# minfenli/refnerf-pl

Measured on AMD Instinct MI355X. Metric: ray-samples/s (4096 rays x 128 samples x 2 levels, Ref-NeRF Blender, eval forward), higher is better.
Workload: dtype f16x2; 1 GPU; blender_refnerf.gin, 4096 rays x 128 samples, 2-level, Model.__call__ eval forward with compute_extras + full ray_history; rays_per_gpu=4096, total_rays=4096, samples_per_level=128, parallelism=ray-tile dp1, n_ranks_seen=1, hip_graph_replay=False

## Files before the change

refnerf-pl_amd/csrc/refnerf_level_bf16.h:

```cpp
#pragma once
#include <type_traits>

#include "refnerf_level_common.h"

namespace rn {

typedef short v2s __attribute__((ext_vector_type(2)));

struct MmBf16 {
  typedef __bf16 t;
  typedef t v8 __attribute__((ext_vector_type(8)));
  typedef t v2 __attribute__((ext_vector_type(2)));
  static __device__ __forceinline__ v16f mfma(v8 a, v8 b, v16f c) { return __builtin_amdgcn_mfma_f32_32x32x16_bf16(a, b, c, 0, 0, 0); }
};
struct MmF16 {
  typedef _Float16 t;
  typedef t v8 __attribute__((ext_vector_type(8)));
  typedef t v2 __attribute__((ext_vector_type(2)));
  static __device__ __forceinline__ v16f mfma(v8 a, v8 b, v16f c) { return __builtin_amdgcn_mfma_f32_32x32x16_f16(a, b, c, 0, 0, 0); }
};
template <typename MM>
__device__ __forceinline__ unsigned cvt_pk_mm(float lo, float hi) {
  typename MM::v2 r = __builtin_convertvector((v2f){lo, hi}, typename MM::v2);
  return __builtin_bit_cast(unsigned, r);
}
constexpr bool ENC_FAST = true;

constexpr int BT = 256;
constexpr int BF_NW = 8;
constexpr int BF_NTHREADS = 64 * BF_NW;
constexpr int BF_RING_SLOTS = 3;
constexpr int BF_RING_BYTES = BF_RING_SLOTS * BF_CHUNK_BYTES;
constexpr int BF_X_BYTES = (IPE_DIM / 8) * BT * 16;
constexpr int AF = 2;
static_assert(AF == 1 || AF == 2 || AF == 4, "the ring index k % AF must stay in phase across 8- and 16-step chunks, and the ring may only run into "
                                             "the next chunk after that chunk's rendezvous (8-step chunks: k >= 4)");

typedef __attribute__((address_space(1))) const void *gptr_t;
typedef __attribute__((address_space(3))) void *lptr_t;

struct Pipe {
  const char *sp;
  unsigned pos;
  unsigned lane_off;
  const char *src;
  const char *src_end;
  char *wbuf;
  const char *xp;
  const char *xps;
  int seq;
  int cur_off, nxt_off, fil_off;
  int dma_left;
  int lane, wave, h;
  long long t_vm, t_bar;
};

#ifdef REFNERF_PROF_WAITS
#define RN_RENDEZVOUS(p) do { \
    long long t0_ = (long long)__builtin_readcyclecounter(); \
    asm volatile("s_waitcnt vmcnt(0)" ::: "memory"); \
    long long t1_ = (long long)__builtin_readcyclecounter(); \
    __syncthreads(); \
    (p).t_vm += t1_ - t0_; \
    (p).t_bar += (long long)__builtin_readcyclecounter() - t1_; } while (0)
#else
#define RN_RENDEZVOUS(p) do { asm volatile("s_waitcnt vmcnt(0)" ::: "memory"); __syncthreads(); } while (0)
#endif
__device__ __forceinline__ void ring_rotate(Pipe &p) {
  const int t = p.cur_off;
  p.cur_off = p.nxt_off;
  p.nxt_off = p.fil_off;
  p.fil_off = t;
}
static_assert(SPPACKED.sp_chunks == 8 + 7 * 16 + 8 + 5 && SPPACKED.total_chunks - SPPACKED.sp_chunks == 8 + 7 * 8 + 8 + 1,
              "the places where level_fwd_split moves the stream position back are written for this chunk sequence");
constexpr int SP_ADV_REWIND = (1 - SPPACKED.sp_chunks) * BF_CHUNK_BYTES;
constexpr int SP_ADV_WRAP = (1 - SPPACKED.total_chunks) * BF_CHUNK_BYTES;
template <bool SPLIT = false>
__device__ __forceinline__ void issue_chunk(Pipe &p, int slot_off, int piece = -1, int adv = BF_CHUNK_BYTES) {
  if (p.dma_left <= 0) return;
  lptr_t dst = (lptr_t)(p.wbuf + slot_off + p.wave * 3072);
  asm volatile("" : "+v"(p.lane_off));
  gptr_t src = (gptr_t)((SPLIT ? p.sp : p.sp + p.pos) + p.lane_off);
  if (piece < 0 || piece == 0) __builtin_amdgcn_global_load_lds(src, dst, 16, 0, 0);
  if (piece < 0 || piece == 1) __builtin_amdgcn_global_load_lds(src, dst, 16, 1024, 0);
  if ((piece < 0 || piece == 2) && p.wave < 5) __builtin_amdgcn_global_load_lds(src, dst, 16, 2048, 0);
  if (piece >= 0 && piece < 2) return;
  p.dma_left -= 1;
  if constexpr (SPLIT) p.sp += adv;
  else {
    p.pos += BF_CHUNK_BYTES;
    p.pos = (p.pos == (unsigned)BFPACKED.chunks_per_pass * BF_CHUNK_BYTES) ? 0u : p.pos;
  }
}
__device__ __forceinline__ void pipe_stream_init(Pipe &p, const void *image, int chunks, int wave, int lane) {
  p.sp = reinterpret_cast<const char *>(image);
  p.pos = 0;
  p.lane_off = (unsigned)(wave * 3072 + lane * 16);
  p.dma_left = wave < 6 ? chunks : 0;
  p.src = nullptr; p.src_end = nullptr; p.seq = 0;
}

template <typename MM>
__device__ __forceinline__ typename MM::v8 lds_frag(const char *q) {
  return *reinterpret_cast<const typename MM::v8 *>(q);
}

__device__ __forceinline__ v16f bias16(const char *w, int h) {
  const v4f *bp = reinterpret_cast<const v4f *>(w + h * 64);
  v4f b0 = bp[0], b1 = bp[1], b2 = bp[2], b3 = bp[3];
  return (v16f){b0[0], b0[1], b0[2], b0[3], b1[0], b1[1], b1[2], b1[3],
                b2[0], b2[1], b2[2], b2[3], b3[0], b3[1], b3[2], b3[3]};
}

template <typename MM, bool RELU>
__device__ __forceinline__ unsigned pack_pair(float lo, float hi) {
  unsigned w = cvt_pk_mm<MM>(lo, hi);
  if (RELU) {
    v2s s = __builtin_bit_cast(v2s, w);
    s = __builtin_elementwise_max(s, (v2s){0, 0});
    w = __builtin_bit_cast(unsigned, s);
  }
  return w;
}

template <typename MM, bool RELU>
__device__ __forceinline__ void pack_acc(const v16f &a, v4uu &f0, v4uu &f1) {
#pragma unroll
  for (int e = 0; e < 4; ++e) {
    f0[e] = pack_pair<MM, RELU>(a[2 * e], a[2 * e + 1]);
    f1[e] = pack_pair<MM, RELU>(a[8 + 2 * e], a[8 + 2 * e + 1]);
  }
}

template <typename MM, int REAL>
__device__ __forceinline__ typename MM::v8 lds_b(const Pipe &p, int kl) {
  const int kk = (kl < REAL) ? kl : kl - REAL;
  return lds_frag<MM>(p.xp + (2 * kk) * BT * 16);
}

struct NoHook { __device__ __forceinline__ void operator()(int) const {} };
template <typename MM, int KIND, int REAL_L, bool FIRST, bool SPLIT = false, typename Hook = NoHook>
__device__ __forceinline__ void bf_chunk(Pipe &p, typename MM::v8 (&a)[AF], const v4uu (&in)[16], const v4uu (&bn)[8], v16f &acc, Hook &&hook = Hook(), int adv = BF_CHUNK_BYTES) {
  typedef typename MM::v8 v8mm;
  constexpr int KS = (KIND == BF_LDS8) ? 8 : 16;
  constexpr int L0 = (KIND == BF_BNLDS) ? 8 : 0;
  constexpr int RDV = KS / 2 - 1;
  static_assert(KS % AF == 0, "ring phase");
  const char *w = p.wbuf + p.cur_off;
  const char *cur = w + 1024 + p.lane * 16;
  const char *nxt = p.wbuf + p.nxt_off + 1024 + p.lane * 16;
  v8mm xr[2];
  if (KIND == BF_LDS8) { xr[0] = lds_b<MM, REAL_L>(p, 0); xr[1] = lds_b<MM, REAL_L>(p, 1); }
  if (FIRST) acc = bias16(w, p.h);
  __builtin_amdgcn_sched_barrier(0);
#pragma unroll
  for (int k = 0; k < KS; ++k) {
    v8mm b;
    const bool lds_step = (KIND == BF_LDS8) || (KIND == BF_BNLDS && k >= 8);
    if (lds_step) b = xr[(k - L0) & 1];
    else if (KIND == BF_REG) b = __builtin_bit_cast(v8mm, in[k]);
    else b = __builtin_bit_cast(v8mm, bn[k & 7]);
    acc = MM::mfma(a[k % AF], b, acc);
    a[k % AF] = (k + AF < KS) ? lds_frag<MM>(cur + (k + AF) * 1024) : lds_frag<MM>(nxt + (k + AF - KS) * 1024);
    hook(k);
    if (KIND == BF_LDS8 || KIND == BF_BNLDS) {
      const int kl2 = k + 2 - L0;
      if (kl2 >= 0 && kl2 < 8 && !(KIND == BF_LDS8 && kl2 < 2)) xr[kl2 & 1] = lds_b<MM, REAL_L>(p, kl2);
    }
    if (k == RDV) {
      RN_RENDEZVOUS(p);
      issue_chunk<SPLIT>(p, p.fil_off, 0);
    }
    if (k == RDV + 2) issue_chunk<SPLIT>(p, p.fil_off, 1);
    if (k == RDV + 4) issue_chunk<SPLIT>(p, p.fil_off, 2, adv);
    __builtin_amdgcn_sched_barrier(0);
  }
  ring_rotate(p);
}

template <bool SPLIT = false>
__device__ __forceinline__ void idle_pass(Pipe &p) {
#pragma unroll 1
  for (int c = 0; c < (SPLIT ? SPPACKED.chunks_per_pass : BFPACKED.chunks_per_pass); ++c) {
    RN_RENDEZVOUS(p);
    issue_chunk<SPLIT>(p, p.fil_off, -1, c + 3 == SPPACKED.sp_chunks ? SP_ADV_REWIND : (c + 3 == SPPACKED.chunks_per_pass ? SP_ADV_WRAP : BF_CHUNK_BYTES));
    ring_rotate(p);
  }
}

template <typename MM, int KIND0, int REAL0>
__device__ __forceinline__ void bf_slice(Pipe &p, typename MM::v8 (&a)[AF], int second, const v4uu (&in)[16], const v4uu (&bn)[8], v16f &acc) {
  bf_chunk<MM, KIND0, REAL0, true>(p, a, in, bn, acc);
  if constexpr (KIND0 == BF_REG) {
    if (second == 1) bf_chunk<MM, BF_LDS8, BF_IPE_REAL_KS, false>(p, a, in, bn, acc);
    else if (second == 2) bf_chunk<MM, BF_BNLDS, BF_DIR_REAL_KS, false>(p, a, in, bn, acc);
  }
}

template <typename MM, int KIND0, int REAL0>
__device__ __forceinline__ void bf_layer(Pipe &p, typename MM::v8 (&a)[AF], int second, const v4uu (&in)[16], const v4uu (&bn)[8], v4uu (&out)[16]) {
#pragma unroll
  for (int ob = 0; ob < 8; ++ob) {
    v16f acc;
    bf_slice<MM, KIND0, REAL0>(p, a, second, in, bn, acc);
    pack_acc<MM, true>(acc, out[2 * ob], out[2 * ob + 1]);
    __builtin_amdgcn_sched_barrier(0);
  }
}

#define RN_STAMPW(A, slot) do { asm volatile("; RNMARK " #slot); if ((A).prof && blockIdx.x == (gridDim.x >> 1) && lane == 0) (A).prof[wave * 32 + (slot)] = (long long)__builtin_readcyclecounter(); } while (0)

constexpr int BF_PS_RING = 512;
template <typename MM, bool RINGPS = false>
__device__ __forceinline__ void level_fwd_mm(const LevelArgs &A) {
  constexpr int PSM = RINGPS ? BF_PS_RING - 1 : 0;
  typedef typename MM::v8 v8mm;
  typedef typename MM::t mm_t;
  extern __shared__ __attribute__((aligned(16))) float smem[];
  const refnerf_level_cfg &cfg = A.cfg;
  const int N = cfg.n_samples;
  const int tid = threadIdx.x, lane = tid & 63;
  const int wave = __builtin_amdgcn_readfirstlane(tid >> 6);
  const int rpw = A.rpw;
  const int ray0 = blockIdx.x * rpw;
  const int n_tot = rpw * N;
  const int n_pass = (n_tot + BT - 1) / BT;

  char *WB = reinterpret_cast<char *>(smem);
  char *Xb = WB + BF_RING_BYTES;
  float *HD = reinterpret_cast<float *>(Xb + BF_X_BYTES);
  float *TD = HD + HD_ROWS * BT;
  float *XP = TD + rpw * (N + 1);
  float *PS = XP + rpw * (N + 1);
  float *PX = PS + (RINGPS ? BF_PS_RING : n_tot) * NPS_EVAL;
  float *NRM = PX + 3 * BT;
  const float *RY = NRM + 8;

  const int h = lane >> 5, n = lane & 31;
  const int col = wave * 32 + n;

  Pipe p;
  pipe_stream_init(p, A.packed, n_pass * BFPACKED.chunks_per_pass, wave, lane);
  p.wbuf = WB;
  p.xp = Xb + (h * BT + col) * 16;
  p.cur_off = 0; p.nxt_off = BF_CHUNK_BYTES; p.fil_off = 2 * BF_CHUNK_BYTES;
  p.lane = lane; p.wave = wave; p.h = h;
  p.t_vm = 0; p.t_bar = 0;
  RN_STAMPW(A, 0);
  issue_chunk(p, p.cur_off);
  issue_chunk(p, p.nxt_off);

  resample_phase<BF_NW, false>(A, reinterpret_cast<float *>(Xb), TD, NRM, ray0, wave, lane);
  RN_STAMPW(A, 1);
  asm volatile("s_waitcnt vmcnt(0)" ::: "memory");
  __syncthreads();
  RN_STAMPW(A, 2);

  if (wave >= BF_NW / 2) __builtin_amdgcn_s_setprio(1);
  v4uu R0[16], R1[16], bn[8];
  v8mm ar[AF];
#pragma unroll
  for (int d = 0; d < AF; ++d) ar[d] = lds_frag<MM>(WB + 1024 + lane * 16 + d * 1024);

  for (int pass0 = 0; pass0 < n_tot; pass0 += BT) {
    int lane_v = lane, col_v = col;
    asm volatile("" : "+v"(lane_v), "+v"(col_v));
    p.lane_off = (unsigned)(wave * 3072 + lane_v * 16);
    auto locate = [&](int &g, int &rl, int &si, bool &valid) {
      int col_l = col, pass_l = pass0;
      asm volatile("" : "+v"(col_l), "+s"(pass_l));
      g = pass_l + col_l;
      rl = g / N;
      si = g - rl * N;
      valid = (g < n_tot) && (ray0 + rl < A.R);
    };
    auto pass_epilogue = [&]() {
      if constexpr (RINGPS) {
        __syncthreads();
        const int end = (pass0 + BT < n_tot) ? pass0 + BT : n_tot;
        int td_o = (int)(TD - smem), xp_o = (int)(XP - smem), ps_o = (int)(PS - smem), nrm_o = (int)(NRM - smem), lane_e = lane, pass_e = pass0;
        int ntot_e = n_tot, ray0_e = ray0, wave_e = wave;
        asm volatile("" : "+s"(td_o), "+s"(xp_o), "+s"(ps_o), "+s"(nrm_o), "+v"(lane_e), "+s"(pass_e), "+s"(ntot_e), "+s"(ray0_e), "+s"(wave_e));
        composite_phase<BF_NW, true, NPS_EVAL, PSM>(A, smem + td_o, smem + xp_o, smem + ps_o, ntot_e, ray0_e, wave_e, lane_e, nullptr, smem + nrm_o,
                                                    pass_e / N, end / N);
      }
    };
    {
      const int g0 = pass0 + wave * 32;
      if (g0 >= n_tot || ray0 + g0 / N >= A.R) { idle_pass(p); pass_epilogue(); continue; }
    }
    auto load_heads = [&](SampleHeads &sh) {
      int g, rl, si; bool valid;
      locate(g, rl, si, valid);
      int ci = col, ro = (valid ? rl : 0) * 12;
      asm volatile("" : "+v"(ci), "+v"(ro));
      float v[3], gp[3], raw_dif[3], raw_tint[3];
#pragma unroll
      for (int i = 0; i < 3; ++i) {
        v[i] = RY[ro + 6 + i];
        gp[i] = HD[(1 + i) * BT + ci];
        raw_dif[i] = HD[(5 + i) * BT + ci];
        raw_tint[i] = HD[(8 + i) * BT + ci];
      }
      sample_heads<ENC_FAST>(cfg, HD[0 * BT + ci], gp, HD[4 * BT + ci], raw_dif, raw_tint, v, sh);
    };

#pragma unroll 1
    for (int phase = 0; phase < 2; ++phase) {
#pragma unroll
      for (int e = 0; e < 16; ++e) { R0[e] = (v4uu){0, 0, 0, 0}; R1[e] = (v4uu){0, 0, 0, 0}; }
      if (phase == 0) {
#pragma unroll
        for (int e = 0; e < 8; ++e) bn[e] = (v4uu){0, 0, 0, 0};
      }
      char *xs = Xb + col * 16;
      if (phase == 0) {
        int g, rl, si; bool valid;
        locate(g, rl, si, valid);
        float o[3], d[3];
        const float *ry = RY + (valid ? rl : 0) * 12;
#pragma unroll
        for (int i = 0; i < 3; ++i) { o[i] = ry[i]; d[i] = ry[3 + i]; }
        float radius = ry[9];
        const float *td = TD + (valid ? rl : 0) * (N + 1);
        float t0 = td[valid ? si : 0], t1 = td[valid ? si + 1 : 1];
        float lm[3], lv[3];
        cast_sample(o, d, radius, t0, t1, cfg.ray_shape, lm, lv);
        if (cfg.disable_integration) { lv[0] = 0.0f; lv[1] = 0.0f; lv[2] = 0.0f; }
        RN_STAMPW(A, 17);
#pragma unroll 1
        for (int qq = 0; qq < 2; ++qq) {
#pragma unroll
          for (int q = 0; q < 3; ++q) {
            v8mm pk;
#pragma unroll
            for (int e = 0; e < 8; ++e) {
              const int kk = q * 8 + e;
              pk[e] = (mm_t)ipe_feature<ENC_FAST>(lm[kk % 3], lv[kk % 3], 8 * qq + kk / 3, h);
            }
            *reinterpret_cast<v8mm *>(xs + (6 * h + 3 * qq + q) * BT * 16) = pk;
          }
        }
        RN_STAMPW(A, 18);
      } else {
        SampleHeads sh;
        load_heads(sh);
        float ide[40];
#pragma unroll
        for (int q = 36; q < 40; ++q) ide[q] = 0.0f;
        if (cfg.dir_enc == REFNERF_DIRENC_POSENC) posenc_eval<ENC_FAST>(sh.refd[0], sh.refd[1], sh.refd[2], h, [&](int q, float val) { ide[q] = val; });
        else ide_eval<ENC_FAST>(sh.refd[0], sh.refd[1], sh.refd[2], sh.rough, h, [&](int q, float val) { ide[q] = val; });
        if (h == 0) ide[36] = sh.dot;
#pragma unroll
        for (int q = 0; q < 5; ++q) {
          v8mm pk;
#pragma unroll
          for (int e = 0; e < 8; ++e) pk[e] = (mm_t)ide[q * 8 + e];
          *reinterpret_cast<v8mm *>(xs + (5 * h + q) * BT * 16) = pk;
        }
      }
      wave_sync();
      RN_STAMPW(A, 3 + phase * 8);

      if (phase == 0) bf_layer<MM, BF_LDS8, BF_IPE_REAL_KS>(p, ar, 0, R0, bn, R0);
      else bf_layer<MM, BF_BNLDS, BF_DIR_REAL_KS>(p, ar, 0, R0, bn, R0);
      RN_STAMPW(A, 4 + phase * 8);
#pragma unroll 1
      for (int it = 0; it < 4; ++it) {
        const int second = (it == 2) ? (phase ? 2 : 1) : 0;
        bf_layer<MM, BF_REG, 0>(p, ar, second, R0, bn, R1);
        if (it < 3) bf_layer<MM, BF_REG, 0>(p, ar, 0, R1, bn, R0);
      }
      RN_STAMPW(A, 5 + phase * 8);
      if (phase == 0) {
#pragma unroll
        for (int ob = 0; ob < 5; ++ob) {
          v16f acc;
          bf_slice<MM, BF_REG, 0>(p, ar, 0, R1, bn, acc);
          if (ob < 4) pack_acc<MM, false>(acc, bn[2 * ob], bn[2 * ob + 1]);
          else {
            int cb = col + 4 * h * BT;
            asm volatile("" : "+v"(cb));
#pragma unroll
            for (int rr = 0; rr < 8; ++rr) {
              int row = (rr & 3) + 8 * (rr >> 2) + 4 * h;
              if (row < HD_ROWS) HD[((rr & 3) + 8 * (rr >> 2)) * BT + cb] = acc[rr];
            }
          }
        }
        wave_sync();
        RN_STAMPW(A, 6);
      } else {
        v16f acc;
        bf_slice<MM, BF_REG, 0>(p, ar, 0, R1, bn, acc);
        float raw_rgb[3];
#pragma unroll
        for (int i = 0; i < 3; ++i) raw_rgb[i] = __shfl(acc[i], n, 64);
        int g_w, rl_w, si_w; bool valid;
        locate(g_w, rl_w, si_w, valid);
        int lane_w = lane, pass_w = pass0;
        asm volatile("" : "+v"(lane_w), "+s"(pass_w));
        if (valid && h == 0) {
          SampleHeads sh;
          load_heads(sh);
          colour_store<ENC_FAST, NPS_EVAL, PSM>(A, sh, raw_rgb, PS, PX, n_tot, g_w, col);
        }
        wave_sync();
        history_flush<NPS_EVAL, PSM>(A, PS, PX, n_tot, pass_w + wave * 32, wave * 32, (size_t)ray0 * N + pass_w + wave * 32, lane_w);
        RN_STAMPW(A, 14);
      }
    }
    __builtin_amdgcn_wave_barrier();
    pass_epilogue();
  }
  asm volatile("s_waitcnt vmcnt(0)" ::: "memory");
  __syncthreads();
  RN_STAMPW(A, 15);
#ifdef REFNERF_PROF_WAITS
  if (A.prof && blockIdx.x == 0 && lane == 0) { A.prof[wave * 32 + 20] = p.t_vm; A.prof[wave * 32 + 21] = p.t_bar; }
#endif

  if constexpr (!RINGPS) composite_phase<BF_NW, true, NPS_EVAL>(A, TD, XP, PS, n_tot, ray0, wave, lane, reinterpret_cast<float *>(WB), NRM);
  RN_STAMPW(A, 16);
}

#ifndef REFNERF_SECONDARY_TU
__global__ __launch_bounds__(BF_NTHREADS) void level_fwd_bf16(const LevelArgs A) { level_fwd_mm<MmBf16>(A); }
__global__ __launch_bounds__(BF_NTHREADS) void level_fwd_f16(const LevelArgs A) { level_fwd_mm<MmF16>(A); }
__global__ __launch_bounds__(BF_NTHREADS) void level_fwd_bf16_ring(const LevelArgs A) { level_fwd_mm<MmBf16, true>(A); }
__global__ __launch_bounds__(BF_NTHREADS) void level_fwd_f16_ring(const LevelArgs A) { level_fwd_mm<MmF16, true>(A); }
#endif

typedef unsigned v2uu __attribute__((ext_vector_type(2)));

__device__ __forceinline__ unsigned pk_f16(float lo, float hi) { return cvt_pk_mm<MmF16>(lo, hi); }
__device__ __forceinline__ void split_pair_f16(float x0, float x1, unsigned &hi, unsigned &lo) {
  hi = pk_f16(x0, x1);
  asm("" : "+v"(hi));
  const MmF16::v2 hv = __builtin_bit_cast(MmF16::v2, hi);
  const _Float16 h0 = hv[0], h1 = hv[1];
  lo = pk_f16(x0 - (float)h0, x1 - (float)h1);
}
typedef _Float16 sq_v8 __attribute__((ext_vector_type(8)));
constexpr int SQ_NF = 4;
constexpr int SQ_XR = 11;
static_assert(SQ_XR != SQ_A && SQ_XR != SQ_B && SQ_XR != SQ_X && SQ_XR != SQ_BN && SQ_XR != SQ_SC, "a kind of its own");
struct SqAcc { v4f t0, t1; };
template <int KIND> constexpr int sq_nm() { return (KIND == SQ_X || KIND == SQ_XR) ? 18 : (KIND == SQ_BN ? 32 : 24); }
template <int KIND> constexpr int sq_np() { return (KIND == SQ_X || KIND == SQ_XR) ? 12 : 16; }
template <int KIND> constexpr int sq_step(int j) { return KIND == SQ_BN ? j / 4 : (KIND == SQ_SC ? j / 3 : j / 6); }
template <int KIND> constexpr int sq_piece(int j) {
  if (KIND == SQ_BN) return 2 * (j / 4) + (j & 1);
  if (KIND == SQ_SC) return 2 * (j / 3) + ((j % 3) == 1 ? 1 : 0);
  return 4 * (j / 6) + ((j % 6) < 4 ? (j % 6) : (j % 6) - 4);
}
template <int KIND> constexpr bool sq_lo(int j) { return KIND == SQ_BN ? (j & 3) >= 2 : (KIND == SQ_SC ? (j % 3) == 2 : (j % 6) >= 4); }
template <int KIND> constexpr int sq_tile(int j) { return KIND == SQ_SC ? 0 : (KIND == SQ_BN ? (j & 1) : ((j % 6) & 1)); }
template <int KIND> constexpr int sq_release(int j) {
  if (KIND == SQ_BN) return (j & 3) >= 2 ? 2 * (j / 4) + ((j & 3) - 2) : -1;
  if (KIND == SQ_SC) return (j % 3) == 1 ? 2 * (j / 3) + 1 : ((j % 3) == 2 ? 2 * (j / 3) : -1);
  const int jj = j % 6, sl = j / 6;
  return jj == 2 ? 4 * sl + 2 : (jj == 3 ? 4 * sl + 3 : (jj == 4 ? 4 * sl : (jj == 5 ? 4 * sl + 1 : -1)));
}
template <int KIND, bool PRE, typename Hook = NoHook>
__device__ __forceinline__ void sq_chunk(Pipe &p, sq_v8 (&fr)[SQ_NF], const v4uu (&in)[16], SqAcc &acc, SqAcc &nacc, Hook &&hook = Hook(), int adv = BF_CHUNK_BYTES) {
  constexpr int NM = sq_nm<KIND>(), NP = sq_np<KIND>();
  constexpr int RDV = NM / 2 - 1;
  const char *w = p.wbuf + p.cur_off;
  const char *cur = w + 1024 + p.lane * 16;
  const char *nxt = p.wbuf + p.nxt_off + 1024 + p.lane * 16;
  sq_v8 xb[2];
  if (KIND == SQ_X) { xb[0] = lds_frag<MmF16>(p.xps); xb[1] = lds_frag<MmF16>(p.xps + (BT / 2) * 16); }
  __builtin_amdgcn_sched_barrier(0);
#pragma unroll
  for (int j = 0; j < NM; ++j) {
    const int sl = sq_step<KIND>(j);
    sq_v8 b;
    if (KIND == SQ_X) b = xb[sq_lo<KIND>(j) ? 1 : 0];
    else b = __builtin_bit_cast(sq_v8, in[2 * ((KIND == SQ_B ? 4 : 0) + sl) + (sq_lo<KIND>(j) ? 1 : 0)]);
    if (sq_tile<KIND>(j)) acc.t1 = __builtin_amdgcn_mfma_f32_16x16x32_f16(fr[sq_piece<KIND>(j) % SQ_NF], b, acc.t1, 0, 0, 0);
    else acc.t0 = __builtin_amdgcn_mfma_f32_16x16x32_f16(fr[sq_piece<KIND>(j) % SQ_NF], b, acc.t0, 0, 0, 0);
    const int rel = sq_release<KIND>(j);
    if (rel >= 0) {
      const int q = rel + SQ_NF;
      fr[rel % SQ_NF] = (q < NP) ? lds_frag<MmF16>(cur + q * 1024) : lds_frag<MmF16>(nxt + (q - NP) * 1024);
    }
    hook(j);
    if (KIND == SQ_X) {
      if ((j % 6) == 3 && sl + 1 < 3) xb[0] = lds_frag<MmF16>(p.xps + (sl + 1) * (4 * BT * 16));
      if ((j % 6) == 5 && sl + 1 < 3) xb[1] = lds_frag<MmF16>(p.xps + (sl + 1) * (4 * BT * 16) + (BT / 2) * 16);
    }
    if (j == RDV) {
      RN_RENDEZVOUS(p);
      issue_chunk<true>(p, p.fil_off, 0);
      if (PRE) {
        const v4f *bp = reinterpret_cast<const v4f *>(p.wbuf + p.nxt_off + (p.lane >> 4) * 16);
        nacc.t0 = bp[0];
        nacc.t1 = bp[4];
      }
    }
    if (j == RDV + 4) issue_chunk<true>(p, p.fil_off, 1);
    if (j == RDV + 8) issue_chunk<true>(p, p.fil_off, 2, adv);
    __builtin_amdgcn_sched_barrier(0);
  }
  ring_rotate(p);
}
__device__ __forceinline__ void sq_epi_piece(const SqAcc &a, int q, v4uu &oh, v4uu &ol) {
  const float y0 = q == 0 ? a.t0[0] : (q == 1 ? a.t0[2] : (q == 2 ? a.t1[0] : a.t1[2]));
  const float y1 = q == 0 ? a.t0[1] : (q == 1 ? a.t0[3] : (q == 2 ? a.t1[1] : a.t1[3]));
  const float x0 = (y0 < 0.0f) ? 0.0f : y0, x1 = (y1 < 0.0f) ? 0.0f : y1;
  unsigned hi, lo;
  split_pair_f16(x0, x1, hi, lo);
  oh[q] = hi;
  ol[q] = lo;
}
template <bool LAYER0>
__device__ __forceinline__ void sq_layer(Pipe &p, sq_v8 (&fr)[SQ_NF], SqAcc (&accs)[2], bool skip, const v4uu (&in)[16], v4uu (&out)[16]) {
#pragma unroll
  for (int ob = 0; ob < 8; ++ob) {
    SqAcc &acc = accs[(ob + 1) & 1];
    SqAcc &prev = accs[ob & 1];
    auto hook = [&](int j) {
      if (ob == 0 || j >= 8 || (j & 1)) return;
      sq_epi_piece(prev, j >> 1, out[2 * ob - 2], out[2 * ob - 1]);
    };
    if constexpr (LAYER0) sq_chunk<SQ_XR, true>(p, fr, in, acc, prev, hook);
    else {
      sq_chunk<SQ_A, false>(p, fr, in, acc, prev, hook);
      sq_chunk<SQ_B, true>(p, fr, in, acc, prev);
      if (skip) sq_chunk<SQ_X, true>(p, fr, in, acc, prev);
    }
  }
#pragma unroll
  for (int q = 0; q < 4; ++q) sq_epi_piece(accs[0], q, out[14], out[15]);
  __builtin_amdgcn_sched_barrier(0);
}
__device__ __forceinline__ void sq_load_ipe_frags(const Pipe &p, v4uu (&in)[16]) {
#pragma unroll
  for (int s = 0; s < 3; ++s) {
    in[2 * s] = __builtin_bit_cast(v4uu, lds_frag<MmF16>(p.xps + s * (4 * BT * 16)));
    in[2 * s + 1] = __builtin_bit_cast(v4uu, lds_frag<MmF16>(p.xps + s * (4 * BT * 16) + (BT / 2) * 16));
  }
}
__device__ __forceinline__ void sq_bias_now(const Pipe &p, SqAcc &acc) {
  const v4f *bp = reinterpret_cast<const v4f *>(p.wbuf + p.cur_off + (p.lane >> 4) * 16);
  acc.t0 = bp[0];
  acc.t1 = bp[4];
}

template <typename MM, int KIND0, int REAL0>
__device__ __forceinline__ void dir_layer(Pipe &p, typename MM::v8 (&a)[AF], int second, const v4uu (&in)[16], const v4uu (&bn)[8], v4uu (&out)[16], int adv6 = BF_CHUNK_BYTES) {
#pragma unroll
  for (int ob = 0; ob < 8; ++ob) {
    v16f acc;
    bf_chunk<MM, KIND0, REAL0, true, true>(p, a, in, bn, acc, NoHook(), ob == 6 ? adv6 : BF_CHUNK_BYTES);
    if constexpr (KIND0 == BF_REG) {
      if (second == 2) bf_chunk<MM, BF_BNLDS, BF_DIR_REAL_KS, false, true>(p, a, in, bn, acc);
    }
    pack_acc<MM, true>(acc, out[2 * ob], out[2 * ob + 1]);
    __builtin_amdgcn_sched_barrier(0);
  }
}

template <bool RINGPS = false>
__device__ __forceinline__ void level_fwd_split(const LevelArgs &A) {
  typedef MmF16 MM;
  constexpr int PSM = RINGPS ? BF_PS_RING - 1 : 0;
  typedef typename MM::v8 v8mm;
  typedef typename MM::t mm_t;
  extern __shared__ __attribute__((aligned(16))) float smem[];
  const refnerf_level_cfg &cfg = A.cfg;
  const int N = cfg.n_samples;
  const int tid = threadIdx.x, lane = tid & 63;
  const int wave = __builtin_amdgcn_readfirstlane(tid >> 6);
  const int rpw = A.rpw;
  const int ray0 = blockIdx.x * rpw;
  const int n_tot = rpw * N;
  const int n_pass = (n_tot + BT - 1) / BT;

  char *WB = reinterpret_cast<char *>(smem);
  char *Xb = WB + BF_RING_BYTES;
  float *HD = reinterpret_cast<float *>(Xb + BF_X_BYTES);
  float *TD = HD + HD_ROWS * BT;
  float *XP = TD + rpw * (N + 1);
  float *PS = XP + rpw * (N + 1);
  float *PX = PS + (RINGPS ? BF_PS_RING : n_tot) * NPS_EVAL;
  float *NRM = PX + 3 * BT;
  const float *RY = NRM + 8;

  const int h = lane >> 5, n = lane & 31;
  const int col = wave * 32 + n;

  Pipe p;
  pipe_stream_init(p, A.packed, n_pass * SPPACKED.chunks_per_pass, wave, lane);
  p.wbuf = WB;
  p.xp = Xb + (h * BT + col) * 16;
  p.xps = Xb + ((lane >> 4) * BT + wave * 16 + (lane & 15)) * 16;
  p.cur_off = 0; p.nxt_off = BF_CHUNK_BYTES; p.fil_off = 2 * BF_CHUNK_BYTES;
  p.lane = lane; p.wave = wave; p.h = h;
  p.t_vm = 0; p.t_bar = 0;
  RN_STAMPW(A, 0);
#ifdef REFNERF_PROF_WAITS
  if (A.prof && blockIdx.x == (gridDim.x >> 1) && lane == 0) A.prof[wave * 32 + 22] = (long long)__builtin_amdgcn_s_memrealtime();
#endif
  issue_chunk<true>(p, p.cur_off);
  issue_chunk<true>(p, p.nxt_off);

  resample_phase<BF_NW, true>(A, reinterpret_cast<float *>(Xb), TD, NRM, ray0, wave, lane);
#pragma clang loop unroll(disable)
  for (int rl = wave; rl < rpw; rl += BF_NW) {
    const int ray = ray0 + rl;
    if (ray >= A.R) break;
    float *RYw = NRM + 8 + rl * 12;
    if (lane < 10) {
      const float val = lane < 3 ? A.rays.d_origins[(size_t)ray * 3 + lane]
                      : lane < 6 ? A.rays.d_directions[(size_t)ray * 3 + lane - 3]
                      : lane < 9 ? A.rays.d_viewdirs[(size_t)ray * 3 + lane - 6] : A.rays.d_radii[ray];
      RYw[lane] = val;
      const float dx = __shfl(val, 3, 64), dy = __shfl(val, 4, 64), dz = __shfl(val, 5, 64);
      if (lane == 0) NRM[rl] = sqrtf((dx * dx + dy * dy) + dz * dz);
    }
  }
  RN_STAMPW(A, 1);
  asm volatile("s_waitcnt vmcnt(0)" ::: "memory");
  __syncthreads();
  RN_STAMPW(A, 2);

  if (wave >= BF_NW / 2) __builtin_amdgcn_s_setprio(1);
  v4uu R0[16], R1[16];
  sq_v8 ar[SQ_NF];
#pragma unroll
  for (int d = 0; d < SQ_NF; ++d) ar[d] = lds_frag<MM>(WB + 1024 + lane * 16 + d * 1024);

  for (int pass0 = 0; pass0 < n_tot; pass0 += BT) {
    int lane_v = lane;
    asm volatile("" : "+v"(lane_v));
    p.lane_off = (unsigned)(wave * 3072 + lane_v * 16);
    auto locate = [&](int &g, int &rl, bool &valid) {
      int col_l = col, pass_l = pass0;
      asm volatile("" : "+v"(col_l), "+s"(pass_l));
      g = pass_l + col_l;
      rl = g / N;
      valid = (g < n_tot) && (ray0 + rl < A.R);
    };
    auto pass_epilogue = [&]() {
      if constexpr (RINGPS) {
        __syncthreads();
        const int end = (pass0 + BT < n_tot) ? pass0 + BT : n_tot;
        int td_o = (int)(TD - smem), xp_o = (int)(XP - smem), ps_o = (int)(PS - smem), nrm_o = (int)(NRM - smem), lane_e = lane, pass_e = pass0;
        int ntot_e = n_tot, ray0_e = ray0, wave_e = wave;
        asm volatile("" : "+s"(td_o), "+s"(xp_o), "+s"(ps_o), "+s"(nrm_o), "+v"(lane_e), "+s"(pass_e), "+s"(ntot_e), "+s"(ray0_e), "+s"(wave_e));
        composite_phase<BF_NW, false, NPS_EVAL, PSM>(A, smem + td_o, smem + xp_o, smem + ps_o, ntot_e, ray0_e, wave_e, lane_e, nullptr, smem + nrm_o,
                                                     pass_e / N, end / N);
      }
    };
    {
      const int g0 = pass0 + wave * 32;
      if (g0 >= n_tot || ray0 + g0 / N >= A.R) { idle_pass<true>(p); pass_epilogue(); continue; }
    }
    auto load_heads = [&](SampleHeads &sh, int &g, bool &valid) {
      int rl;
      locate(g, rl, valid);
      int ci = col, ro = (valid ? rl : 0) * 12;
      asm volatile("" : "+v"(ci), "+v"(ro));
      float v[3], gp[3], raw_dif[3], raw_tint[3];
#pragma unroll
      for (int i = 0; i < 3; ++i) {
        v[i] = RY[ro + 6 + i];
        gp[i] = HD[(1 + i) * BT + ci];
        raw_dif[i] = HD[(5 + i) * BT + ci];
        raw_tint[i] = HD[(8 + i) * BT + ci];
      }
      sample_heads<false>(cfg, HD[0 * BT + ci], gp, HD[4 * BT + ci], raw_dif, raw_tint, v, sh);
    };

    v4uu bn0[4];
    auto heads = [&](auto RUN, v4uu (&bn)[8]) {
      constexpr int run = decltype(RUN)::value;
      SqAcc ha[2];
      sq_bias_now(p, ha[1]);
#pragma unroll
      for (int ob = 0; ob < 5; ++ob) {
        SqAcc &acc = ha[(ob + 1) & 1];
        if (ob < 4) {
          sq_chunk<SQ_BN, true>(p, ar, R1, acc, ha[ob & 1], NoHook(), (run == 0 && ob == 2) ? SP_ADV_REWIND : BF_CHUNK_BYTES);
#pragma unroll
          for (int e = 0; e < 4; ++e) {
            const unsigned pk = e == 0 ? pk_f16(acc.t0[0], acc.t0[1]) : (e == 1 ? pk_f16(acc.t0[2], acc.t0[3])
                              : (e == 2 ? pk_f16(acc.t1[0], acc.t1[1]) : pk_f16(acc.t1[2], acc.t1[3])));
            if (run == 0) bn0[ob][e] = pk;
            else {
              const v2uu r = __builtin_amdgcn_permlane16_swap(bn0[ob][e], pk, false, false);
              bn[2 * ob][e] = r[0];
              bn[2 * ob + 1][e] = r[1];
            }
          }
        } else {
          sq_chunk<SQ_SC, false>(p, ar, R1, acc, ha[ob & 1]);
          const int bq = lane_v >> 4;
          int csl = wave * 32 + 16 * run + (lane_v & 15) + 4 * bq * BT;
          asm volatile("" : "+v"(csl));
#pragma unroll
          for (int i = 0; i < 4; ++i)
            if (4 * bq + i < HD_ROWS) HD[i * BT + csl] = acc.t0[i];
        }
      }
      wave_sync();
    };
    typedef std::integral_constant<int, 0> Run0;
    typedef std::integral_constant<int, 1> Run1;

#pragma unroll 1
    for (int phase = 0; phase < 2; ++phase) {
#pragma unroll
      for (int e = 0; e < 16; ++e) { R0[e] = (v4uu){0, 0, 0, 0}; R1[e] = (v4uu){0, 0, 0, 0}; }
      {
      const int i16 = lane_v & 15, part = lane_v >> 4;
      const int hb = part >> 1, qq = part & 1;
      const int cs = wave * 32 + 16 * phase + i16;
      const int gs = pass0 + cs;
      const int rls = gs / N, sis = gs - rls * N;
      const bool vs = (gs < n_tot) && (ray0 + rls < A.R);
      float o[3], d[3];
      const float *ry = RY + (vs ? rls : 0) * 12;
#pragma unroll
      for (int i = 0; i < 3; ++i) { o[i] = ry[i]; d[i] = ry[3 + i]; }
      const float radius = ry[9];
      const float *td = TD + (vs ? rls : 0) * (N + 1);
      const float t0 = td[vs ? sis : 0], t1 = td[vs ? sis + 1 : 1];
      float lm[3], lv[3];
      cast_sample(o, d, radius, t0, t1, cfg.ray_shape, lm, lv);
      if (cfg.disable_integration) { lv[0] = 0.0f; lv[1] = 0.0f; lv[2] = 0.0f; }
      char *xw = Xb + (wave * 16 + i16) * 16;
      RN_STAMPW(A, 17);
      float sc = qq ? 256.0f : 1.0f, sc2 = qq ? 65536.0f : 1.0f;
      char *xq = xw + (6 * hb + 3 * qq) * BT * 16;
#pragma clang loop unroll(disable)
      for (int dp = 0; dp < 4; ++dp) {
        const float sc_odd = sc * 2.0f, sc2_odd = sc2 * 4.0f;
#pragma unroll
        for (int a = 0; a < 3; ++a) {
          float f[2];
#pragma unroll
          for (int u = 0; u < 2; ++u) {
            const int k6 = 2 * a + u, odd = k6 / 3, b3 = k6 - 3 * odd;
            f[u] = ipe_feature_split_sc(lm[b3], lv[b3], odd ? sc_odd : sc, odd ? sc2_odd : sc2, hb);
          }
          unsigned whi, wlo;
          split_pair_f16(f[0], f[1], whi, wlo);
          const int t = 3 * dp + a;
          char *dst = xq + (t >> 2) * BT * 16 + (t & 3) * 4;
          *reinterpret_cast<unsigned *>(dst) = whi;
          *reinterpret_cast<unsigned *>(dst + (BT / 2) * 16) = wlo;
        }
        sc *= 4.0f;
        sc2 *= 16.0f;
      }
      }
      RN_STAMPW(A, 18);
      wave_sync();
      RN_STAMPW(A, 3 + phase * 4);
      if (phase == 0) {
#pragma unroll
        for (int d = AF; d < SQ_NF; ++d) ar[d] = lds_frag<MM>(p.wbuf + p.cur_off + 1024 + lane_v * 16 + d * 1024);
      }
      SqAcc accs[2];
      sq_bias_now(p, accs[1]);
      sq_load_ipe_frags(p, R1);
      sq_layer<true>(p, ar, accs, false, R1, R0);
#pragma unroll
      for (int e = 0; e < 6; ++e) R1[e] = (v4uu){0, 0, 0, 0};
      RN_STAMPW(A, 4 + phase * 4);
#pragma unroll 1
      for (int it = 0; it < 4; ++it) {
        sq_layer<false>(p, ar, accs, it == 2, R0, R1);
        if (it < 3) sq_layer<false>(p, ar, accs, false, R1, R0);
      }
      RN_STAMPW(A, 5 + phase * 4);
      if (phase == 0) {
        v4uu none[8];
        heads(Run0(), none);
        RN_STAMPW(A, 6);
      }
    }
    v4uu bn[8];
    heads(Run1(), bn);
    RN_STAMPW(A, 10);
#pragma unroll
    for (int e = 0; e < 16; ++e) { R0[e] = (v4uu){0, 0, 0, 0}; R1[e] = (v4uu){0, 0, 0, 0}; }
    {
    const int h4 = RINGPS ? (fresh_lane() >> 5) : h;
    char *xs = Xb + col * 16;
    {
      SampleHeads sh;
      int g4; bool valid4;
      load_heads(sh, g4, valid4);
      if (valid4 && h4 == 0) heads_store<NPS_EVAL, PSM>(sh, PS, PX, g4, RINGPS ? wave * 32 + (fresh_lane() & 31) : col);
      float ide[40];
#pragma unroll
      for (int q = 36; q < 40; ++q) ide[q] = 0.0f;
      if (cfg.dir_enc == REFNERF_DIRENC_POSENC) posenc_eval<false, true>(sh.refd[0], sh.refd[1], sh.refd[2], h4, [&](int q, float val) { ide[q] = val; });
      else ide_eval<false>(sh.refd[0], sh.refd[1], sh.refd[2], sh.rough, h4, [&](int q, float val) { ide[q] = val; });
      if (h4 == 0) ide[36] = sh.dot;
#pragma unroll
      for (int q = 0; q < 5; ++q) {
        v8mm pk;
#pragma unroll
        for (int e = 0; e < 8; ++e) pk[e] = (mm_t)ide[q * 8 + e];
        *reinterpret_cast<v8mm *>(xs + (5 * h4 + q) * BT * 16) = pk;
      }
    }
    wave_sync();
    RN_STAMPW(A, 11);
    v8mm (&ad)[AF] = reinterpret_cast<v8mm (&)[AF]>(ar);
    dir_layer<MM, BF_BNLDS, BF_DIR_REAL_KS>(p, ad, 0, R0, bn, R0);
    RN_STAMPW(A, 12);
#pragma unroll 1
    for (int it = 0; it < 4; ++it) {
      dir_layer<MM, BF_REG, 0>(p, ad, (it == 2) ? 2 : 0, R0, bn, R1, it == 3 ? SP_ADV_WRAP : BF_CHUNK_BYTES);
      if (it < 3) dir_layer<MM, BF_REG, 0>(p, ad, 0, R1, bn, R0);
    }
    RN_STAMPW(A, 13);
    v16f acc;
    bf_chunk<MM, BF_REG, 0, true, true>(p, ad, R1, bn, acc);
    float raw_rgb[3];
    const int lane6 = RINGPS ? fresh_lane() : lane;
    const int n6 = RINGPS ? (lane6 & 31) : n, h6 = RINGPS ? (lane6 >> 5) : h;
#pragma unroll
    for (int i = 0; i < 3; ++i) raw_rgb[i] = __shfl(acc[i], n6, 64);
    int g_w, rl_w; bool valid;
    locate(g_w, rl_w, valid);
    int lane_w = lane6, pass_w = pass0;
    asm volatile("" : "+v"(lane_w), "+s"(pass_w));
    if (valid) {
      int ci = RINGPS ? wave * 32 + n6 : col, pr = ps_row<PSM>(g_w) * NPS_EVAL;
      asm volatile("" : "+v"(ci), "+v"(pr));
      float tint[3], raw_dif[3];
#pragma unroll
      for (int i = 0; i < 3; ++i) { tint[i] = PS[pr + PS_TINT + i]; raw_dif[i] = HD[(5 + i) * BT + ci]; }
      int half = h6;
      asm volatile("" : "+v"(half));
      colour_store_halves<NPS_EVAL, PSM, true>(A, half, tint, raw_dif, raw_rgb, PS, g_w);
    }
    wave_sync();
    history_flush<NPS_EVAL, PSM>(A, PS, PX, n_tot, pass_w + wave * 32, wave * 32, (size_t)ray0 * N + pass_w + wave * 32, lane_w);
    RN_STAMPW(A, 14);
    }
    __builtin_amdgcn_wave_barrier();
    pass_epilogue();
  }
  asm volatile("s_waitcnt vmcnt(0)" ::: "memory");
  __syncthreads();
  RN_STAMPW(A, 15);
#ifdef REFNERF_PROF_WAITS
  if (A.prof && blockIdx.x == (gridDim.x >> 1) && lane == 0) {
    A.prof[wave * 32 + 20] = p.t_vm; A.prof[wave * 32 + 21] = p.t_bar;
    A.prof[wave * 32 + 23] = (long long)__builtin_amdgcn_s_memrealtime();
  }
#endif
  if constexpr (!RINGPS) composite_phase<BF_NW, false, NPS_EVAL>(A, TD, XP, PS, n_tot, ray0, wave, lane, reinterpret_cast<float *>(WB), NRM);
  RN_STAMPW(A, 16);
}

#ifndef REFNERF_SECONDARY_TU
__global__ __launch_bounds__(BF_NTHREADS) void level_fwd_f16x2(const LevelArgs A) { level_fwd_split<false>(A); }
__global__ __launch_bounds__(BF_NTHREADS) void level_fwd_f16x2_ring(const LevelArgs A) { level_fwd_split<true>(A); }
#endif

__device__ __forceinline__ int ipe_col_of_kprime(int kp) { return kp; }

}
```

Baseline: 282.7 million ray-samples/s.

## Deepen weight-fragment register ring to eight slots in MLP trunk chunks

Widens the LDS weight-fragment prefetch ring from SQ_NF to eight slots for most trunk output blocks, with a compile-time checker confirming every slot is refilled before it is read and that next-chunk slots are only read after the rendezvous. The last block drops back to the shallower ring so the depth matches what the code after the trunk expects. The aim is more prefetch distance between LDS fragment loads and the MFMAs that consume them, hiding LDS latency. The cost is extra VGPRs, which may lower occupancy or cause spills, and the rendezvous point moves earlier for 12-piece chunks.

```diff
diff --git a/refnerf-pl_amd/csrc/refnerf_level_bf16.h b/refnerf-pl_amd/csrc/refnerf_level_bf16.h
--- a/refnerf-pl_amd/csrc/refnerf_level_bf16.h
+++ b/refnerf-pl_amd/csrc/refnerf_level_bf16.h
@@ -463,15 +463,47 @@
   const int jj = j % 6, sl = j / 6;
   return jj == 2 ? 4 * sl + 2 : (jj == 3 ? 4 * sl + 3 : (jj == 4 ? 4 * sl : (jj == 5 ? 4 * sl + 1 : -1)));
 }
-template <int KIND, bool PRE, typename Hook = NoHook>
-__device__ __forceinline__ void sq_chunk(Pipe &p, sq_v8 (&fr)[SQ_NF], const v4uu (&in)[16], SqAcc &acc, SqAcc &nacc, Hook &&hook = Hook(), int adv = BF_CHUNK_BYTES) {
-  constexpr int NM = sq_nm<KIND>(), NP = sq_np<KIND>();
-  constexpr int RDV = NM / 2 - 1;
+constexpr int SQ_NFE = 8;
+struct SqRefill { int slot, piece; bool nxt; };
+template <int KIND, int D> constexpr SqRefill sq_refill(int rel) {
+  constexpr int NP = sq_np<KIND>();
+  if (NP == 12 && D == 8) return rel < 4 ? SqRefill{rel, rel + 8, false} : (rel < 8 ? SqRefill{rel, rel, true} : SqRefill{rel - 8, rel - 8, true});
+  return rel + D < NP ? SqRefill{rel % D, rel + D, false} : SqRefill{rel % D, rel + D - NP, true};
+}
+template <int KIND, int D> constexpr int sq_rdv() { return sq_nm<KIND>() / 2 - ((sq_np<KIND>() == 12 && D == 8) ? 2 : 1); }
+template <int KIND, int D, int E> constexpr bool sq_ring_ok() {
+  constexpr int NM = sq_nm<KIND>(), NP = sq_np<KIND>(), RDV = sq_rdv<KIND, D>();
+  if (!((D == SQ_NF || D == SQ_NFE) && (E == SQ_NF || E == SQ_NFE)) || RDV < 0 || RDV + 8 >= NM) return false;
+  int slot[SQ_NFE] = {-1, -1, -1, -1, -1, -1, -1, -1};
+  for (int d = 0; d < (E < D ? E : D); ++d) slot[d] = d;
+  for (int d = E; d < D; ++d) slot[d] = d;
+  for (int j = 0; j < NM; ++j) {
+    const int q = sq_piece<KIND>(j);
+    if (q >= NP || slot[q % D] != q) return false;
+    const int rel = sq_release<KIND>(j);
+    if (rel < 0) continue;
+    const SqRefill r = sq_refill<KIND, D>(rel);
+    if (r.slot < 0 || r.slot >= D || slot[r.slot] != rel) return false;
+    for (int i = j + 1; i < NM; ++i) if (sq_piece<KIND>(i) == rel) return false;
+    if (r.nxt && j <= RDV) return false;
+    if (!r.nxt && r.piece >= NP) return false;
+    slot[r.slot] = r.nxt ? 100 + r.piece : r.piece;
+  }
+  for (int d = 0; d < D; ++d) if (slot[d] != 100 + d) return false;
+  return true;
+}
+template <int KIND, bool PRE, int D = SQ_NF, int E = D, typename Hook = NoHook>
+__device__ __forceinline__ void sq_chunk(Pipe &p, sq_v8 (&fr)[SQ_NFE], const v4uu (&in)[16], SqAcc &acc, SqAcc &nacc, Hook &&hook = Hook(), int adv = BF_CHUNK_BYTES) {
+  constexpr int NM = sq_nm<KIND>();
+  constexpr int RDV = sq_rdv<KIND, D>();
+  static_assert(sq_ring_ok<KIND, D, E>(), "piece ring: a slot read before it is filled, or the next chunk's slot read before the rendezvous");
   const char *w = p.wbuf + p.cur_off;
   const char *cur = w + 1024 + p.lane * 16;
   const char *nxt = p.wbuf + p.nxt_off + 1024 + p.lane * 16;
   sq_v8 xb[2];
   if (KIND == SQ_X) { xb[0] = lds_frag<MmF16>(p.xps); xb[1] = lds_frag<MmF16>(p.xps + (BT / 2) * 16); }
+#pragma unroll
+  for (int d = E; d < D; ++d) fr[d] = lds_frag<MmF16>(cur + d * 1024);
   __builtin_amdgcn_sched_barrier(0);
 #pragma unroll
   for (int j = 0; j < NM; ++j) {
@@ -479,12 +511,12 @@
     sq_v8 b;
     if (KIND == SQ_X) b = xb[sq_lo<KIND>(j) ? 1 : 0];
     else b = __builtin_bit_cast(sq_v8, in[2 * ((KIND == SQ_B ? 4 : 0) + sl) + (sq_lo<KIND>(j) ? 1 : 0)]);
-    if (sq_tile<KIND>(j)) acc.t1 = __builtin_amdgcn_mfma_f32_16x16x32_f16(fr[sq_piece<KIND>(j) % SQ_NF], b, acc.t1, 0, 0, 0);
-    else acc.t0 = __builtin_amdgcn_mfma_f32_16x16x32_f16(fr[sq_piece<KIND>(j) % SQ_NF], b, acc.t0, 0, 0, 0);
+    if (sq_tile<KIND>(j)) acc.t1 = __builtin_amdgcn_mfma_f32_16x16x32_f16(fr[sq_piece<KIND>(j) % D], b, acc.t1, 0, 0, 0);
+    else acc.t0 = __builtin_amdgcn_mfma_f32_16x16x32_f16(fr[sq_piece<KIND>(j) % D], b, acc.t0, 0, 0, 0);
     const int rel = sq_release<KIND>(j);
     if (rel >= 0) {
-      const int q = rel + SQ_NF;
-      fr[rel % SQ_NF] = (q < NP) ? lds_frag<MmF16>(cur + q * 1024) : lds_frag<MmF16>(nxt + (q - NP) * 1024);
+      const SqRefill r = sq_refill<KIND, D>(rel);
+      fr[r.slot] = lds_frag<MmF16>((r.nxt ? nxt : cur) + r.piece * 1024);
     }
     hook(j);
     if (KIND == SQ_X) {
@@ -515,23 +547,35 @@
   oh[q] = hi;
   ol[q] = lo;
 }
+template <bool LAYER0> constexpr int sq_depth(int ob) { return (LAYER0 || ob < 7) ? SQ_NFE : SQ_NF; }
+constexpr int SQ_TRUNK_ENTRY = sq_depth<true>(7) < sq_depth<false>(7) ? sq_depth<true>(7) : sq_depth<false>(7);
+template <bool LAYER0, int OB>
+__device__ __forceinline__ void sq_slice(Pipe &p, sq_v8 (&fr)[SQ_NFE], SqAcc (&accs)[2], bool skip, const v4uu (&in)[16], v4uu (&out)[16]) {
+  constexpr int D = sq_depth<LAYER0>(OB);
+  constexpr int E = OB > 0 ? sq_depth<LAYER0>(OB > 0 ? OB - 1 : 0) : (LAYER0 ? SQ_NF : SQ_TRUNK_ENTRY);
+  SqAcc &acc = accs[(OB + 1) & 1];
+  SqAcc &prev = accs[OB & 1];
+  auto hook = [&](int j) {
+    if (OB == 0 || j >= 8 || (j & 1)) return;
+    sq_epi_piece(prev, j >> 1, out[OB > 0 ? 2 * OB - 2 : 0], out[OB > 0 ? 2 * OB - 1 : 0]);
+  };
+  if constexpr (LAYER0) sq_chunk<SQ_XR, true, D, E>(p, fr, in, acc, prev, hook);
+  else {
+    sq_chunk<SQ_A, false, D, E>(p, fr, in, acc, prev, hook);
+    sq_chunk<SQ_B, true, D>(p, fr, in, acc, prev);
+    if (skip) sq_chunk<SQ_X, true, D>(p, fr, in, acc, prev);
+  }
+}
 template <bool LAYER0>
-__device__ __forceinline__ void sq_layer(Pipe &p, sq_v8 (&fr)[SQ_NF], SqAcc (&accs)[2], bool skip, const v4uu (&in)[16], v4uu (&out)[16]) {
-#pragma unroll
-  for (int ob = 0; ob < 8; ++ob) {
-    SqAcc &acc = accs[(ob + 1) & 1];
-    SqAcc &prev = accs[ob & 1];
-    auto hook = [&](int j) {
-      if (ob == 0 || j >= 8 || (j & 1)) return;
-      sq_epi_piece(prev, j >> 1, out[2 * ob - 2], out[2 * ob - 1]);
-    };
-    if constexpr (LAYER0) sq_chunk<SQ_XR, true>(p, fr, in, acc, prev, hook);
-    else {
-      sq_chunk<SQ_A, false>(p, fr, in, acc, prev, hook);
-      sq_chunk<SQ_B, true>(p, fr, in, acc, prev);
-      if (skip) sq_chunk<SQ_X, true>(p, fr, in, acc, prev);
-    }
-  }
+__device__ __forceinline__ void sq_layer(Pipe &p, sq_v8 (&fr)[SQ_NFE], SqAcc (&accs)[2], bool skip, const v4uu (&in)[16], v4uu (&out)[16]) {
+  sq_slice<LAYER0, 0>(p, fr, accs, skip, in, out);
+  sq_slice<LAYER0, 1>(p, fr, accs, skip, in, out);
+  sq_slice<LAYER0, 2>(p, fr, accs, skip, in, out);
+  sq_slice<LAYER0, 3>(p, fr, accs, skip, in, out);
+  sq_slice<LAYER0, 4>(p, fr, accs, skip, in, out);
+  sq_slice<LAYER0, 5>(p, fr, accs, skip, in, out);
+  sq_slice<LAYER0, 6>(p, fr, accs, skip, in, out);
+  sq_slice<LAYER0, 7>(p, fr, accs, skip, in, out);
 #pragma unroll
   for (int q = 0; q < 4; ++q) sq_epi_piece(accs[0], q, out[14], out[15]);
   __builtin_amdgcn_sched_barrier(0);
@@ -629,7 +673,7 @@
 
   if (wave >= BF_NW / 2) __builtin_amdgcn_s_setprio(1);
   v4uu R0[16], R1[16];
-  sq_v8 ar[SQ_NF];
+  sq_v8 ar[SQ_NFE];
 #pragma unroll
   for (int d = 0; d < SQ_NF; ++d) ar[d] = lds_frag<MM>(WB + 1024 + lane * 16 + d * 1024);
 
```

Result: no change. 284.1 million ray-samples/s, median of 6 (+0.5%).
